# eikehmueller/IncompressibleEulerHDG

Measured on AMD Instinct MI355X. Metric: million DOF-updates/sec (HDG-IMEX k=2, 1024^2 tri mesh), higher is better.
Workload: dtype f64

## Files before the change

incompressibleeulerhdg_amd/csrc/hdg_trace_tile.hpp:

```cpp
#pragma once
#include <hip/hip_runtime.h>

namespace hdg {

template <int K>
struct TraceTile {
  static constexpr int NL = Dim<K>::NL, NT = 3 * NL;
  static constexpr int TW = 16, TH = 8, NTHREADS = 256;
  static constexpr int W2 = TW + 4, H2 = TH + 4, N2 = W2 * H2;
  static constexpr int WPE_POST = K == 1 ? 5 : (K == 2 ? 4 : (K == 3 ? 3 : 1));
  static constexpr int W3 = TW + 6, H3 = TH + 6, N3 = W3 * H3;
  static constexpr int W1 = TW + 2, H1 = TH + 2, N1 = W1 * H1;
  static constexpr int KMAX = (N2 + NTHREADS - 1) / NTHREADS;
};

template <int K, int RW, int RH>
__device__ __forceinline__ void lds_trace_stencil(const double* __restrict__ A, int li, int lj, bool in_x, bool in_y, bool below,
                                                  bool left, const DevTables& T, double* own, double* yH, double* yV, double* yD) {
  constexpr int NL = Dim<K>::NL, NT = 3 * NL;
  auto at = [&](int t, int m, int dj, int di) { return A[((t * NL + m) * RH + (lj + dj)) * RW + (li + di)]; };
  double uA[NT], uB[NT], uC[NT];
#pragma unroll
  for (int m = 0; m < NL; m++) {
    own[m] = at(0, m, 0, 0); own[NL + m] = at(2, m, 0, 0); own[2 * NL + m] = at(1, m, 0, 0);
    uA[m] = at(0, m, 1, 0); uA[2 * NL + m] = at(1, m, 0, 1);
    uB[NL + m] = at(2, m, -1, 0); uB[2 * NL + m] = at(1, m, -1, 1);
    uC[m] = at(0, m, 1, -1); uC[NL + m] = at(2, m, 0, -1);
    yH[m] = yV[m] = yD[m] = 0.0;
  }
  const bool vL = in_x && in_y, vB = in_x && below, vW = in_y && left;
#pragma unroll
  for (int m = 0; m < NL; m++) {
    if (!in_x) own[m] = 0.0;
    if (!vL) own[NL + m] = 0.0;
    if (!in_y) own[2 * NL + m] = 0.0;
    uA[NL + m] = own[NL + m];
    uB[m] = own[m];
    uC[2 * NL + m] = own[2 * NL + m];
  }
  const double* __restrict__ SL = T.SK[0];
  const double* __restrict__ SU = T.SK[1];
  if (vL) {
    mv_acc_ld<NL, NT>(SL + 0 * NL * NT, NT, own, yH, -1.0);
    mv_acc_ld<NL, NT>(SL + 1 * NL * NT, NT, own, yD, -1.0);
    mv_acc_ld<NL, NT>(SL + 2 * NL * NT, NT, own, yV, -1.0);
    mv_acc_ld<NL, NT>(SU + 1 * NL * NT, NT, uA, yD, -1.0);
  }
  if (vB) mv_acc_ld<NL, NT>(SU + 0 * NL * NT, NT, uB, yH, -1.0);
  if (vW) mv_acc_ld<NL, NT>(SU + 2 * NL * NT, NT, uC, yV, -1.0);
}

#define HDG_TILE_OF_BLOCK                                              \
  const int tiles_per_xcd_ = (int)(gridDim.x >> 3);                    \
  const int tile_v = (int)(blockIdx.x & 7) * tiles_per_xcd_ + (int)(blockIdx.x >> 3); \
  if (tile_v >= ntx * nty) return;                                     \
  const int tile_y = tile_v / ntx, tile_x = tile_v - tile_y * ntx;
struct CornerInfo {
  bool exists, in_x, in_y, below, left;
  bool own_x;
  int vH, vV;
  long o;
};
struct TileRows {
  int jlo, jhi, rlo, rhi;
};
__device__ __forceinline__ CornerInfo corner_info(const Geo& g, const TileRows& tr, int i, int j) {
  CornerInfo c;
  const int gj = g.joff + j;
  if (g.px) {
    c.exists = gj >= 0 && gj <= g.nyg && j >= tr.rlo && j < tr.rhi;
    c.own_x = i >= 0 && i < g.nx;
    const int iw = i < 0 ? i + g.nx : (i >= g.nx ? i - g.nx : i);
    c.in_x = c.exists;
    c.in_y = c.exists && gj < g.nyg;
    c.below = gj > 0;
    c.left = true;
    c.vH = gj == 0 ? 1 : (gj == g.nyg ? 2 : 0);
    c.vV = 0;
    c.o = (long)(j + GH) * g.P + iw;
    return c;
  }
  c.exists = i >= 0 && i <= g.nx && gj >= 0 && gj <= g.nyg && j >= tr.rlo && j < tr.rhi;
  c.own_x = true;
  c.in_x = c.exists && i < g.nx;
  c.in_y = c.exists && gj < g.nyg;
  c.below = gj > 0;
  c.left = i > 0;
  c.vH = gj == 0 ? 1 : (gj == g.nyg ? 2 : 0);
  c.vV = i == 0 ? 1 : (i == g.nx ? 2 : 0);
  c.o = (long)(j + GH) * g.P + i;
  return c;
}
template <int NL>
__device__ __forceinline__ void load_corner(const double* __restrict__ v, const Geo& g, const CornerInfo& c, double* e) {
#pragma unroll
  for (int m = 0; m < NL; m++) {
    e[m] = c.in_x ? v[((long)0 * NL + m) * g.G + c.o] : 0.0;
    e[NL + m] = (c.in_x && c.in_y) ? v[((long)2 * NL + m) * g.G + c.o] : 0.0;
    e[2 * NL + m] = c.in_y ? v[((long)1 * NL + m) * g.G + c.o] : 0.0;
  }
}
template <int NL>
__device__ __forceinline__ void store_corner(double* __restrict__ v, const Geo& g, const CornerInfo& c, const double* e) {
#pragma unroll
  for (int m = 0; m < NL; m++) {
    v[((long)0 * NL + m) * g.G + c.o] = c.in_x ? e[m] : 0.0;
    v[((long)2 * NL + m) * g.G + c.o] = (c.in_x && c.in_y) ? e[NL + m] : 0.0;
    v[((long)1 * NL + m) * g.G + c.o] = c.in_y ? e[2 * NL + m] : 0.0;
  }
}
template <int NL>
__device__ __forceinline__ void corner_dinv(const DevTables& T, const CornerInfo& c, double sc, const double* r, double* z) {
#pragma unroll
  for (int q = 0; q < 3 * NL; q++) z[q] = 0.0;
  mv_acc_ld<NL, NL>(T.trDinv[0][0], NL, r, z, sc);
  mv_acc_ld<NL, NL>(T.trDinv[2][0], NL, r + NL, z + NL, sc);
  mv_acc_ld<NL, NL>(T.trDinv[1][0], NL, r + 2 * NL, z + 2 * NL, sc);
  if (c.vH != 0) {
#pragma unroll
    for (int q = 0; q < NL; q++) z[q] = 0.0;
    mv_acc_ld<NL, NL>(T.trDinv[0][c.vH], NL, r, z, sc);
  }
  if (c.vV != 0) {
#pragma unroll
    for (int q = 0; q < NL; q++) z[2 * NL + q] = 0.0;
    mv_acc_ld<NL, NL>(T.trDinv[1][c.vV], NL, r + 2 * NL, z + 2 * NL, sc);
  }
}
template <int NL>
__device__ __forceinline__ int plane_of(int q) { return q < NL ? q : (q < 2 * NL ? 2 * NL + (q - NL) : NL + (q - 2 * NL)); }

template <int K>
__global__ __launch_bounds__(TraceTile<K>::NTHREADS) void k_trace_pre_tile(int ntx, int nty, Geo g, TileRows tr, DevTables T, const double* __restrict__ r, double c0, double c1,
                                                         double c2, double* __restrict__ z_out, double* __restrict__ res_out) {
  typedef TraceTile<K> TT;
  constexpr int NL = TT::NL, NT = TT::NT, TW = TT::TW, TH = TT::TH, W2 = TT::W2, H2 = TT::H2, W1 = TT::W1, H1 = TT::H1, KMAX = TT::KMAX;
  __shared__ double Ds[NT * TT::N2];
  __shared__ double Zs[NT * TT::N1];
  HDG_TILE_OF_BLOCK
  const int i0 = tile_x * TW, j0 = tr.jlo + tile_y * TH;
  double rr[KMAX][NT], dd[KMAX][NT];
#pragma unroll
  for (int k = 0; k < KMAX; k++) {
    const int idx = threadIdx.x + k * TT::NTHREADS;
    if (idx < TT::N2) {
      const int lj = idx / W2, li = idx - lj * W2;
      const int jc = j0 - 2 + lj;
      const CornerInfo c = corner_info(g, tr, i0 - 2 + li, jc);
      load_corner<NL>(r, g, c, rr[k]);
      corner_dinv<NL>(T, c, c0, rr[k], dd[k]);
#pragma unroll
      for (int q = 0; q < NT; q++) Ds[(plane_of<NL>(q) * H2 + lj) * W2 + li] = dd[k][q];
    }
  }
  __syncthreads();
#pragma unroll
  for (int k = 0; k < KMAX; k++) {
    const int idx = threadIdx.x + k * TT::NTHREADS;
    if (idx < TT::N2) {
      const int lj = idx / W2, li = idx - lj * W2;
      if (li >= 1 && li < W2 - 1 && lj >= 1 && lj < H2 - 1) {
        const int jc = j0 - 2 + lj;
        const CornerInfo c = corner_info(g, tr, i0 - 2 + li, jc);
        double z[NT];
#pragma unroll
        for (int q = 0; q < NT; q++) z[q] = 0.0;
        if (c.exists) {
          double own[NT], y[3][NL], r1[NT], zz[NT];
          lds_trace_stencil<K, W2, H2>(Ds, li, lj, c.in_x, c.in_y, c.below, c.left, T, own, y[0], y[1], y[2]);
#pragma unroll
          for (int m = 0; m < NL; m++) {
            r1[m] = rr[k][m] - y[0][m];
            r1[NL + m] = rr[k][NL + m] - y[2][m];
            r1[2 * NL + m] = rr[k][2 * NL + m] - y[1][m];
          }
          corner_dinv<NL>(T, c, c2, r1, zz);
#pragma unroll
          for (int q = 0; q < NT; q++) z[q] = dd[k][q] + fma(c1, dd[k][q], zz[q]);
        }
#pragma unroll
        for (int q = 0; q < NT; q++) Zs[(plane_of<NL>(q) * H1 + (lj - 1)) * W1 + (li - 1)] = z[q];
        if (c.exists && c.own_x && li >= 2 && li < W2 - 2 && lj >= 2 && lj < H2 - 2 && jc < tr.jhi) store_corner<NL>(z_out, g, c, z);
      }
    }
  }
  __syncthreads();
#pragma unroll
  for (int k = 0; k < KMAX; k++) {
    const int idx = threadIdx.x + k * TT::NTHREADS;
    if (idx < TT::N2) {
      const int lj = idx / W2, li = idx - lj * W2;
      if (li >= 2 && li < W2 - 2 && lj >= 2 && lj < H2 - 2) {
        const int jc = j0 - 2 + lj;
        const CornerInfo c = corner_info(g, tr, i0 - 2 + li, jc);
        if (c.exists && c.own_x && jc < tr.jhi) {
          double own[NT], y[3][NL], res[NT];
          lds_trace_stencil<K, W1, H1>(Zs, li - 1, lj - 1, c.in_x, c.in_y, c.below, c.left, T, own, y[0], y[1], y[2]);
#pragma unroll
          for (int m = 0; m < NL; m++) {
            res[m] = rr[k][m] - y[0][m];
            res[NL + m] = rr[k][NL + m] - y[2][m];
            res[2 * NL + m] = rr[k][2 * NL + m] - y[1][m];
          }
          store_corner<NL>(res_out, g, c, res);
        }
      }
    }
  }
}

template <int K, bool DOTS>
__global__ __launch_bounds__(TraceTile<K>::NTHREADS) __attribute__((amdgpu_waves_per_eu(TraceTile<K>::WPE_POST))) void k_trace_post_tile(int ntx, int nty, Geo g, TileRows tr, DevTables T, const double* __restrict__ z_in, const double* __restrict__ r,
                                                          const double* __restrict__ xc, double sH, double sV, double sD, double c0,
                                                          double c1, double c2, double* __restrict__ z_out, double* __restrict__ w_out,
                                                          double* __restrict__ part) {
  typedef TraceTile<K> TT;
  constexpr int NL = TT::NL, NT = TT::NT, TW = TT::TW, TH = TT::TH, W2 = TT::W2, H2 = TT::H2, W3 = TT::W3, H3 = TT::H3, KMAX = TT::KMAX;
  __shared__ double Zs[NT * TT::N3];
  __shared__ double Ds[NT * TT::N2];
  HDG_TILE_OF_BLOCK
  const int i0 = tile_x * TW, j0 = tr.jlo + tile_y * TH;
  const int st = g.nx + 1;
  for (int idx = threadIdx.x; idx < TT::N3; idx += TT::NTHREADS) {
    const int lj = idx / W3, li = idx - lj * W3;
    const int i = i0 - 3 + li, j = j0 - 3 + lj;
    const CornerInfo c = corner_info(g, tr, i, j);
    double z[NT];
    load_corner<NL>(z_in, g, c, z);
    if (c.exists && g.px) {
      const int n = g.nx, m = g.nx, jg = g.pj0 + j;
      const int iw = i < 0 ? i + n : (i >= n ? i - n : i), i1 = iw + 1 == n ? 0 : iw + 1;
      const int jw = jg < 0 ? jg + m : (jg >= m ? jg - m : jg), j1 = jw + 1 == m ? 0 : jw + 1;
      const double v00 = xc[(long)jw * n + iw], v10 = xc[(long)jw * n + i1], v01 = xc[(long)j1 * n + iw];
      edge_prolong(v00, v10, sH, z);
      if (c.in_y) edge_prolong(v10, v01, sD, z + NL);
      if (c.in_y) edge_prolong(v00, v01, sV, z + 2 * NL);
    } else if (c.exists) {
      const long J = g.joff + j;
      const double v00 = xc[J * st + i];
      const double v10 = c.in_x ? xc[J * st + i + 1] : 0.0, v01 = c.in_y ? xc[(J + 1) * st + i] : 0.0;
      if (c.in_x) edge_prolong(v00, v10, sH, z);
      if (c.in_x && c.in_y) edge_prolong(v10, v01, sD, z + NL);
      if (c.in_y) edge_prolong(v00, v01, sV, z + 2 * NL);
    }
#pragma unroll
    for (int q = 0; q < NT; q++) Zs[(plane_of<NL>(q) * H3 + lj) * W3 + li] = z[q];
  }
  double r0[KMAX][NT];
#pragma unroll
  for (int k = 0; k < KMAX; k++) {
    const int idx = threadIdx.x + k * TT::NTHREADS;
    const int lj = idx / W2, li = idx - lj * W2;
    CornerInfo c = corner_info(g, tr, i0 - 2 + li, j0 - 2 + lj);
    if (idx >= TT::N2) c.in_x = c.in_y = false;
    load_corner<NL>(r, g, c, r0[k]);
  }
  __syncthreads();
  double dots[5] = {0.0, 0.0, 0.0, 0.0, 0.0};
#pragma unroll
  for (int k = 0; k < KMAX; k++) {
    const int idx = threadIdx.x + k * TT::NTHREADS;
    if (idx < TT::N2) {
      const int lj = idx / W2, li = idx - lj * W2;
      const int jc = j0 - 2 + lj;
      const CornerInfo c = corner_info(g, tr, i0 - 2 + li, jc);
      double d0[NT];
#pragma unroll
      for (int q = 0; q < NT; q++) d0[q] = 0.0;
      if (c.exists) {
        double own[NT], y[3][NL];
        lds_trace_stencil<K, W3, H3>(Zs, li + 1, lj + 1, c.in_x, c.in_y, c.below, c.left, T, own, y[0], y[1], y[2]);
#pragma unroll
        for (int m = 0; m < NL; m++) {
          r0[k][m] -= y[0][m];
          r0[k][NL + m] -= y[2][m];
          r0[k][2 * NL + m] -= y[1][m];
        }
        corner_dinv<NL>(T, c, c0, r0[k], d0);
      }
#pragma unroll
      for (int q = 0; q < NT; q++) Ds[(plane_of<NL>(q) * H2 + lj) * W2 + li] = d0[q];
    }
  }
  __syncthreads();
#pragma unroll
  for (int k = 0; k < KMAX; k++) {
    const int idx = threadIdx.x + k * TT::NTHREADS;
    if (idx < TT::N2) {
      const int lj = idx / W2, li = idx - lj * W2;
      if (li >= 1 && li < W2 - 1 && lj >= 1 && lj < H2 - 1) {
        const int jc = j0 - 2 + lj;
        const CornerInfo c = corner_info(g, tr, i0 - 2 + li, jc);
        double z2[NT];
#pragma unroll
        for (int q = 0; q < NT; q++) z2[q] = 0.0;
        if (c.exists) {
          double own[NT], y[3][NL], r1[NT], zz[NT];
          lds_trace_stencil<K, W2, H2>(Ds, li, lj, c.in_x, c.in_y, c.below, c.left, T, own, y[0], y[1], y[2]);
#pragma unroll
          for (int m = 0; m < NL; m++) {
            r1[m] = r0[k][m] - y[0][m];
            r1[NL + m] = r0[k][NL + m] - y[2][m];
            r1[2 * NL + m] = r0[k][2 * NL + m] - y[1][m];
          }
          corner_dinv<NL>(T, c, c2, r1, zz);
#pragma unroll
          for (int q = 0; q < NT; q++) {
            const double z1 = Zs[(plane_of<NL>(q) * H3 + (lj + 1)) * W3 + (li + 1)] + own[q];
            z2[q] = z1 + fma(c1, own[q], zz[q]);
          }
        }
#pragma unroll
        for (int q = 0; q < NT; q++) Zs[(plane_of<NL>(q) * H3 + (lj + 1)) * W3 + (li + 1)] = z2[q];
        if (c.exists && c.own_x && li >= 2 && li < W2 - 2 && lj >= 2 && lj < H2 - 2 && jc < tr.jhi) store_corner<NL>(z_out, g, c, z2);
      }
    }
  }
  if (!w_out) return;
  double rr3[KMAX][NT];
  if (DOTS) {
#pragma unroll
    for (int k = 0; k < KMAX; k++) {
      const int idx = threadIdx.x + k * TT::NTHREADS;
      const int lj = idx / W2, li = idx - lj * W2;
      const int jc = j0 - 2 + lj;
      CornerInfo c = corner_info(g, tr, i0 - 2 + li, jc);
      if (!(idx < TT::N2 && li >= 2 && li < W2 - 2 && lj >= 2 && lj < H2 - 2 && c.exists && c.own_x && jc < tr.jhi)) c.in_x = c.in_y = false;
      load_corner<NL>(r, g, c, rr3[k]);
    }
  }
  __syncthreads();
#pragma unroll
  for (int k = 0; k < KMAX; k++) {
    const int idx = threadIdx.x + k * TT::NTHREADS;
    if (idx < TT::N2) {
      const int lj = idx / W2, li = idx - lj * W2;
      if (li >= 2 && li < W2 - 2 && lj >= 2 && lj < H2 - 2) {
        const int jc = j0 - 2 + lj;
        const CornerInfo c = corner_info(g, tr, i0 - 2 + li, jc);
        if (c.exists && c.own_x && jc < tr.jhi) {
          double own[NT], y[3][NL], w[NT];
          lds_trace_stencil<K, W3, H3>(Zs, li + 1, lj + 1, c.in_x, c.in_y, c.below, c.left, T, own, y[0], y[1], y[2]);
#pragma unroll
          for (int m = 0; m < NL; m++) { w[m] = y[0][m]; w[NL + m] = y[2][m]; w[2 * NL + m] = y[1][m]; }
          store_corner<NL>(w_out, g, c, w);
          if (DOTS) {
            const double* rr = rr3[k];
            dots[0] += sH * own[0] + sD * own[NL] + sV * own[2 * NL];
            dots[4] += sH * rr[0] + sD * rr[NL] + sV * rr[2 * NL];
#pragma unroll
            for (int q = 0; q < NT; q++) {
              const double zq = own[q];
              dots[1] = fma(zq, rr[q], dots[1]);
              dots[2] = fma(zq, zq, dots[2]);
              dots[3] = fma(zq, w[q], dots[3]);
            }
          }
        }
      }
    }
  }
  if (DOTS) {
    __shared__ double sm[TT::NTHREADS / 64][5];
    const int lane = threadIdx.x & 63, wv = threadIdx.x >> 6;
#pragma unroll
    for (int q = 0; q < 5; q++) {
      const double sv = wave_sum(dots[q]);
      if (lane == 0) sm[wv][q] = sv;
    }
    __syncthreads();
    if (threadIdx.x < 5) {
      double sv = 0.0;
      for (int w2 = 0; w2 < TT::NTHREADS / 64; w2++) sv += sm[w2][threadIdx.x];
      part[(long)threadIdx.x * (ntx * nty) + tile_v] = sv;
    }
  }
}

}
```

Before: 830.6.

## Remap tile corners to threads interior-first so inner stages use whole waves

Replaces the row-major halo-region-to-thread mapping with an interior-first, then ring-1, then ring-2 ordering, one corner per thread (N2=240 fits in 256 threads). Later stages, which only touch the halo-1 or interior region, now sit in contiguous waves, and whole waves that have no work skip a stage through a wave-uniform check. The per-thread KMAX arrays and their loops are dropped, which may lower register pressure. The dot-product reduction is rerouted through LDS in row-major order, presumably to keep the summation order deterministic, at the cost of an extra barrier and LDS traffic.

```diff
diff --git a/incompressibleeulerhdg_amd/csrc/hdg_tile_map.hpp b/incompressibleeulerhdg_amd/csrc/hdg_tile_map.hpp
--- /dev/null
+++ b/incompressibleeulerhdg_amd/csrc/hdg_tile_map.hpp
@@ -0,0 +1,34 @@
+#pragma once
+
+namespace hdg {
+
+template <int K>
+struct TileShape {
+  static constexpr int TW = 16, TH = 8;
+};
+
+struct TileCorner {
+  int li, lj;
+};
+
+template <int TW, int TH>
+constexpr TileCorner ring_corner(int r, int p) {
+  const int w = TW + 2 * r, h = TH + 2 * r, o = 2 - r;
+  if (p < 2 * w) {
+    const int top = p >= w ? 1 : 0;
+    return TileCorner{o + p - top * w, o + top * (h - 1)};
+  }
+  p -= 2 * w;
+  const int right = p >= h - 2 ? 1 : 0;
+  return TileCorner{o + right * (w - 1), o + 1 + p - right * (h - 2)};
+}
+
+template <int TW, int TH>
+constexpr TileCorner tile_corner(int idx) {
+  constexpr int N0 = TW * TH, N1 = (TW + 2) * (TH + 2);
+  if (idx < N0) return TileCorner{2 + idx % TW, 2 + idx / TW};
+  if (idx < N1) return ring_corner<TW, TH>(1, idx - N0);
+  return ring_corner<TW, TH>(2, idx - N1);
+}
+
+}
diff --git a/incompressibleeulerhdg_amd/csrc/hdg_trace_tile.hpp b/incompressibleeulerhdg_amd/csrc/hdg_trace_tile.hpp
--- a/incompressibleeulerhdg_amd/csrc/hdg_trace_tile.hpp
+++ b/incompressibleeulerhdg_amd/csrc/hdg_trace_tile.hpp
@@ -1,17 +1,33 @@
 #pragma once
 #include <hip/hip_runtime.h>
+
+#include "hdg_tile_map.hpp"
 
 namespace hdg {
 
 template <int K>
 struct TraceTile {
   static constexpr int NL = Dim<K>::NL, NT = 3 * NL;
-  static constexpr int TW = 16, TH = 8, NTHREADS = 256;
+  static constexpr int TW = TileShape<K>::TW, TH = TileShape<K>::TH, NTHREADS = 256;
+  static constexpr int N0 = TW * TH;
   static constexpr int W2 = TW + 4, H2 = TH + 4, N2 = W2 * H2;
   static constexpr int WPE_POST = K == 1 ? 5 : (K == 2 ? 4 : (K == 3 ? 3 : 1));
   static constexpr int W3 = TW + 6, H3 = TH + 6, N3 = W3 * H3;
   static constexpr int W1 = TW + 2, H1 = TH + 2, N1 = W1 * H1;
-  static constexpr int KMAX = (N2 + NTHREADS - 1) / NTHREADS;
+  static_assert(N2 <= NTHREADS && N3 <= 2 * NTHREADS, "one corner of the halo-2 region per thread, two trips over the halo-3 region");
+};
+
+template <int K>
+struct TileWave {
+  int idx, li, lj;
+  int first;
+  __device__ __forceinline__ TileWave() {
+    idx = (int)threadIdx.x;
+    first = __builtin_amdgcn_readfirstlane(idx) & ~63;
+    const TileCorner c = tile_corner<TraceTile<K>::TW, TraceTile<K>::TH>(idx);
+    li = c.li; lj = c.lj;
+  }
+  __device__ __forceinline__ bool runs(int n) const { return first < n; }
 };
 
 template <int K, int RW, int RH>
@@ -134,77 +150,57 @@
 __global__ __launch_bounds__(TraceTile<K>::NTHREADS) void k_trace_pre_tile(int ntx, int nty, Geo g, TileRows tr, DevTables T, const double* __restrict__ r, double c0, double c1,
                                                          double c2, double* __restrict__ z_out, double* __restrict__ res_out) {
   typedef TraceTile<K> TT;
-  constexpr int NL = TT::NL, NT = TT::NT, TW = TT::TW, TH = TT::TH, W2 = TT::W2, H2 = TT::H2, W1 = TT::W1, H1 = TT::H1, KMAX = TT::KMAX;
+  constexpr int NL = TT::NL, NT = TT::NT, TW = TT::TW, TH = TT::TH, W2 = TT::W2, H2 = TT::H2, W1 = TT::W1, H1 = TT::H1;
   __shared__ double Ds[NT * TT::N2];
   __shared__ double Zs[NT * TT::N1];
   HDG_TILE_OF_BLOCK
   const int i0 = tile_x * TW, j0 = tr.jlo + tile_y * TH;
-  double rr[KMAX][NT], dd[KMAX][NT];
-#pragma unroll
-  for (int k = 0; k < KMAX; k++) {
-    const int idx = threadIdx.x + k * TT::NTHREADS;
-    if (idx < TT::N2) {
-      const int lj = idx / W2, li = idx - lj * W2;
-      const int jc = j0 - 2 + lj;
-      const CornerInfo c = corner_info(g, tr, i0 - 2 + li, jc);
-      load_corner<NL>(r, g, c, rr[k]);
-      corner_dinv<NL>(T, c, c0, rr[k], dd[k]);
-#pragma unroll
-      for (int q = 0; q < NT; q++) Ds[(plane_of<NL>(q) * H2 + lj) * W2 + li] = dd[k][q];
-    }
-  }
-  __syncthreads();
-#pragma unroll
-  for (int k = 0; k < KMAX; k++) {
-    const int idx = threadIdx.x + k * TT::NTHREADS;
-    if (idx < TT::N2) {
-      const int lj = idx / W2, li = idx - lj * W2;
-      if (li >= 1 && li < W2 - 1 && lj >= 1 && lj < H2 - 1) {
-        const int jc = j0 - 2 + lj;
-        const CornerInfo c = corner_info(g, tr, i0 - 2 + li, jc);
-        double z[NT];
-#pragma unroll
-        for (int q = 0; q < NT; q++) z[q] = 0.0;
-        if (c.exists) {
-          double own[NT], y[3][NL], r1[NT], zz[NT];
-          lds_trace_stencil<K, W2, H2>(Ds, li, lj, c.in_x, c.in_y, c.below, c.left, T, own, y[0], y[1], y[2]);
-#pragma unroll
-          for (int m = 0; m < NL; m++) {
-            r1[m] = rr[k][m] - y[0][m];
-            r1[NL + m] = rr[k][NL + m] - y[2][m];
-            r1[2 * NL + m] = rr[k][2 * NL + m] - y[1][m];
-          }
-          corner_dinv<NL>(T, c, c2, r1, zz);
-#pragma unroll
-          for (int q = 0; q < NT; q++) z[q] = dd[k][q] + fma(c1, dd[k][q], zz[q]);
+  const TileWave<K> tw;
+  const int idx = tw.idx, li = tw.li, lj = tw.lj, jc = j0 - 2 + lj;
+  const CornerInfo c = corner_info(g, tr, i0 - 2 + li, jc);
+  double rr[NT], dd[NT];
+  if (idx < TT::N2) {
+    load_corner<NL>(r, g, c, rr);
+    corner_dinv<NL>(T, c, c0, rr, dd);
+#pragma unroll
+    for (int q = 0; q < NT; q++) Ds[(plane_of<NL>(q) * H2 + lj) * W2 + li] = dd[q];
+  }
+  __syncthreads();
+  if (tw.runs(TT::N1)) {
+    if (idx < TT::N1) {
+      double z[NT];
+#pragma unroll
+      for (int q = 0; q < NT; q++) z[q] = 0.0;
+      if (c.exists) {
+        double own[NT], y[3][NL], r1[NT], zz[NT];
+        lds_trace_stencil<K, W2, H2>(Ds, li, lj, c.in_x, c.in_y, c.below, c.left, T, own, y[0], y[1], y[2]);
+#pragma unroll
+        for (int m = 0; m < NL; m++) {
+          r1[m] = rr[m] - y[0][m];
+          r1[NL + m] = rr[NL + m] - y[2][m];
+          r1[2 * NL + m] = rr[2 * NL + m] - y[1][m];
         }
-#pragma unroll
-        for (int q = 0; q < NT; q++) Zs[(plane_of<NL>(q) * H1 + (lj - 1)) * W1 + (li - 1)] = z[q];
-        if (c.exists && c.own_x && li >= 2 && li < W2 - 2 && lj >= 2 && lj < H2 - 2 && jc < tr.jhi) store_corner<NL>(z_out, g, c, z);
-      }
-    }
-  }
-  __syncthreads();
-#pragma unroll
-  for (int k = 0; k < KMAX; k++) {
-    const int idx = threadIdx.x + k * TT::NTHREADS;
-    if (idx < TT::N2) {
-      const int lj = idx / W2, li = idx - lj * W2;
-      if (li >= 2 && li < W2 - 2 && lj >= 2 && lj < H2 - 2) {
-        const int jc = j0 - 2 + lj;
-        const CornerInfo c = corner_info(g, tr, i0 - 2 + li, jc);
-        if (c.exists && c.own_x && jc < tr.jhi) {
-          double own[NT], y[3][NL], res[NT];
-          lds_trace_stencil<K, W1, H1>(Zs, li - 1, lj - 1, c.in_x, c.in_y, c.below, c.left, T, own, y[0], y[1], y[2]);
-#pragma unroll
-          for (int m = 0; m < NL; m++) {
-            res[m] = rr[k][m] - y[0][m];
-            res[NL + m] = rr[k][NL + m] - y[2][m];
-            res[2 * NL + m] = rr[k][2 * NL + m] - y[1][m];
-          }
-          store_corner<NL>(res_out, g, c, res);
-        }
-      }
+        corner_dinv<NL>(T, c, c2, r1, zz);
+#pragma unroll
+        for (int q = 0; q < NT; q++) z[q] = dd[q] + fma(c1, dd[q], zz[q]);
+      }
+#pragma unroll
+      for (int q = 0; q < NT; q++) Zs[(plane_of<NL>(q) * H1 + (lj - 1)) * W1 + (li - 1)] = z[q];
+      if (c.exists && c.own_x && idx < TT::N0 && jc < tr.jhi) store_corner<NL>(z_out, g, c, z);
+    }
+  }
+  __syncthreads();
+  if (tw.runs(TT::N0)) {
+    if (idx < TT::N0 && c.exists && c.own_x && jc < tr.jhi) {
+      double own[NT], y[3][NL], res[NT];
+      lds_trace_stencil<K, W1, H1>(Zs, li - 1, lj - 1, c.in_x, c.in_y, c.below, c.left, T, own, y[0], y[1], y[2]);
+#pragma unroll
+      for (int m = 0; m < NL; m++) {
+        res[m] = rr[m] - y[0][m];
+        res[NL + m] = rr[NL + m] - y[2][m];
+        res[2 * NL + m] = rr[2 * NL + m] - y[1][m];
+      }
+      store_corner<NL>(res_out, g, c, res);
     }
   }
 }
@@ -215,14 +211,20 @@
                                                           double c1, double c2, double* __restrict__ z_out, double* __restrict__ w_out,
                                                           double* __restrict__ part) {
   typedef TraceTile<K> TT;
-  constexpr int NL = TT::NL, NT = TT::NT, TW = TT::TW, TH = TT::TH, W2 = TT::W2, H2 = TT::H2, W3 = TT::W3, H3 = TT::H3, KMAX = TT::KMAX;
+  constexpr int NL = TT::NL, NT = TT::NT, TW = TT::TW, TH = TT::TH, W2 = TT::W2, H2 = TT::H2, W3 = TT::W3, H3 = TT::H3;
   __shared__ double Zs[NT * TT::N3];
   __shared__ double Ds[NT * TT::N2];
   HDG_TILE_OF_BLOCK
   const int i0 = tile_x * TW, j0 = tr.jlo + tile_y * TH;
   const int st = g.nx + 1;
-  for (int idx = threadIdx.x; idx < TT::N3; idx += TT::NTHREADS) {
-    const int lj = idx / W3, li = idx - lj * W3;
+  const TileWave<K> tw;
+  const int idx = tw.idx;
+  constexpr int REST = TT::N3 - TT::NTHREADS;
+#pragma unroll
+  for (int trip = 0; trip < 2; trip++) {
+    const int idx3 = idx + trip * REST;
+    if (trip == 1 && idx3 < TT::NTHREADS) continue;
+    const int lj = idx3 / W3, li = idx3 - lj * W3;
     const int i = i0 - 3 + li, j = j0 - 3 + lj;
     const CornerInfo c = corner_info(g, tr, i, j);
     double z[NT];
@@ -246,135 +248,115 @@
 #pragma unroll
     for (int q = 0; q < NT; q++) Zs[(plane_of<NL>(q) * H3 + lj) * W3 + li] = z[q];
   }
-  double r0[KMAX][NT];
-#pragma unroll
-  for (int k = 0; k < KMAX; k++) {
-    const int idx = threadIdx.x + k * TT::NTHREADS;
-    const int lj = idx / W2, li = idx - lj * W2;
-    CornerInfo c = corner_info(g, tr, i0 - 2 + li, j0 - 2 + lj);
-    if (idx >= TT::N2) c.in_x = c.in_y = false;
-    load_corner<NL>(r, g, c, r0[k]);
+  const int li = tw.li, lj = tw.lj, jc = j0 - 2 + lj;
+  const CornerInfo c = corner_info(g, tr, i0 - 2 + li, jc);
+  double r0[NT];
+  {
+    CornerInfo cl = c;
+    if (idx >= TT::N2) cl.in_x = cl.in_y = false;
+    load_corner<NL>(r, g, cl, r0);
   }
   __syncthreads();
   double dots[5] = {0.0, 0.0, 0.0, 0.0, 0.0};
-#pragma unroll
-  for (int k = 0; k < KMAX; k++) {
-    const int idx = threadIdx.x + k * TT::NTHREADS;
-    if (idx < TT::N2) {
-      const int lj = idx / W2, li = idx - lj * W2;
-      const int jc = j0 - 2 + lj;
-      const CornerInfo c = corner_info(g, tr, i0 - 2 + li, jc);
-      double d0[NT];
-#pragma unroll
-      for (int q = 0; q < NT; q++) d0[q] = 0.0;
+  if (idx < TT::N2) {
+    double d0[NT];
+#pragma unroll
+    for (int q = 0; q < NT; q++) d0[q] = 0.0;
+    if (c.exists) {
+      double own[NT], y[3][NL];
+      lds_trace_stencil<K, W3, H3>(Zs, li + 1, lj + 1, c.in_x, c.in_y, c.below, c.left, T, own, y[0], y[1], y[2]);
+#pragma unroll
+      for (int m = 0; m < NL; m++) {
+        r0[m] -= y[0][m];
+        r0[NL + m] -= y[2][m];
+        r0[2 * NL + m] -= y[1][m];
+      }
+      corner_dinv<NL>(T, c, c0, r0, d0);
+    }
+#pragma unroll
+    for (int q = 0; q < NT; q++) Ds[(plane_of<NL>(q) * H2 + lj) * W2 + li] = d0[q];
+  }
+  __syncthreads();
+  if (tw.runs(TT::N1)) {
+    if (idx < TT::N1) {
+      double z2[NT];
+#pragma unroll
+      for (int q = 0; q < NT; q++) z2[q] = 0.0;
       if (c.exists) {
-        double own[NT], y[3][NL];
-        lds_trace_stencil<K, W3, H3>(Zs, li + 1, lj + 1, c.in_x, c.in_y, c.below, c.left, T, own, y[0], y[1], y[2]);
+        double own[NT], y[3][NL], r1[NT], zz[NT];
+        lds_trace_stencil<K, W2, H2>(Ds, li, lj, c.in_x, c.in_y, c.below, c.left, T, own, y[0], y[1], y[2]);
 #pragma unroll
         for (int m = 0; m < NL; m++) {
-          r0[k][m] -= y[0][m];
-          r0[k][NL + m] -= y[2][m];
-          r0[k][2 * NL + m] -= y[1][m];
+          r1[m] = r0[m] - y[0][m];
+          r1[NL + m] = r0[NL + m] - y[2][m];
+          r1[2 * NL + m] = r0[2 * NL + m] - y[1][m];
         }
-        corner_dinv<NL>(T, c, c0, r0[k], d0);
-      }
-#pragma unroll
-      for (int q = 0; q < NT; q++) Ds[(plane_of<NL>(q) * H2 + lj) * W2 + li] = d0[q];
-    }
-  }
-  __syncthreads();
-#pragma unroll
-  for (int k = 0; k < KMAX; k++) {
-    const int idx = threadIdx.x + k * TT::NTHREADS;
-    if (idx < TT::N2) {
-      const int lj = idx / W2, li = idx - lj * W2;
-      if (li >= 1 && li < W2 - 1 && lj >= 1 && lj < H2 - 1) {
-        const int jc = j0 - 2 + lj;
-        const CornerInfo c = corner_info(g, tr, i0 - 2 + li, jc);
-        double z2[NT];
-#pragma unroll
-        for (int q = 0; q < NT; q++) z2[q] = 0.0;
-        if (c.exists) {
-          double own[NT], y[3][NL], r1[NT], zz[NT];
-          lds_trace_stencil<K, W2, H2>(Ds, li, lj, c.in_x, c.in_y, c.below, c.left, T, own, y[0], y[1], y[2]);
-#pragma unroll
-          for (int m = 0; m < NL; m++) {
-            r1[m] = r0[k][m] - y[0][m];
-            r1[NL + m] = r0[k][NL + m] - y[2][m];
-            r1[2 * NL + m] = r0[k][2 * NL + m] - y[1][m];
-          }
-          corner_dinv<NL>(T, c, c2, r1, zz);
-#pragma unroll
-          for (int q = 0; q < NT; q++) {
-            const double z1 = Zs[(plane_of<NL>(q) * H3 + (lj + 1)) * W3 + (li + 1)] + own[q];
-            z2[q] = z1 + fma(c1, own[q], zz[q]);
-          }
+        corner_dinv<NL>(T, c, c2, r1, zz);
+#pragma unroll
+        for (int q = 0; q < NT; q++) {
+          const double z1 = Zs[(plane_of<NL>(q) * H3 + (lj + 1)) * W3 + (li + 1)] + own[q];
+          z2[q] = z1 + fma(c1, own[q], zz[q]);
         }
-#pragma unroll
-        for (int q = 0; q < NT; q++) Zs[(plane_of<NL>(q) * H3 + (lj + 1)) * W3 + (li + 1)] = z2[q];
-        if (c.exists && c.own_x && li >= 2 && li < W2 - 2 && lj >= 2 && lj < H2 - 2 && jc < tr.jhi) store_corner<NL>(z_out, g, c, z2);
-      }
+      }
+#pragma unroll
+      for (int q = 0; q < NT; q++) Zs[(plane_of<NL>(q) * H3 + (lj + 1)) * W3 + (li + 1)] = z2[q];
+      if (c.exists && c.own_x && idx < TT::N0 && jc < tr.jhi) store_corner<NL>(z_out, g, c, z2);
     }
   }
   if (!w_out) return;
-  double rr3[KMAX][NT];
-  if (DOTS) {
-#pragma unroll
-    for (int k = 0; k < KMAX; k++) {
-      const int idx = threadIdx.x + k * TT::NTHREADS;
-      const int lj = idx / W2, li = idx - lj * W2;
-      const int jc = j0 - 2 + lj;
-      CornerInfo c = corner_info(g, tr, i0 - 2 + li, jc);
-      if (!(idx < TT::N2 && li >= 2 && li < W2 - 2 && lj >= 2 && lj < H2 - 2 && c.exists && c.own_x && jc < tr.jhi)) c.in_x = c.in_y = false;
-      load_corner<NL>(r, g, c, rr3[k]);
-    }
-  }
-  __syncthreads();
-#pragma unroll
-  for (int k = 0; k < KMAX; k++) {
-    const int idx = threadIdx.x + k * TT::NTHREADS;
-    if (idx < TT::N2) {
-      const int lj = idx / W2, li = idx - lj * W2;
-      if (li >= 2 && li < W2 - 2 && lj >= 2 && lj < H2 - 2) {
-        const int jc = j0 - 2 + lj;
-        const CornerInfo c = corner_info(g, tr, i0 - 2 + li, jc);
-        if (c.exists && c.own_x && jc < tr.jhi) {
-          double own[NT], y[3][NL], w[NT];
-          lds_trace_stencil<K, W3, H3>(Zs, li + 1, lj + 1, c.in_x, c.in_y, c.below, c.left, T, own, y[0], y[1], y[2]);
-#pragma unroll
-          for (int m = 0; m < NL; m++) { w[m] = y[0][m]; w[NL + m] = y[2][m]; w[2 * NL + m] = y[1][m]; }
-          store_corner<NL>(w_out, g, c, w);
-          if (DOTS) {
-            const double* rr = rr3[k];
-            dots[0] += sH * own[0] + sD * own[NL] + sV * own[2 * NL];
-            dots[4] += sH * rr[0] + sD * rr[NL] + sV * rr[2 * NL];
-#pragma unroll
-            for (int q = 0; q < NT; q++) {
-              const double zq = own[q];
-              dots[1] = fma(zq, rr[q], dots[1]);
-              dots[2] = fma(zq, zq, dots[2]);
-              dots[3] = fma(zq, w[q], dots[3]);
-            }
-          }
+  const bool run3 = tw.runs(TT::N0);
+  const bool live3 = idx < TT::N0 && c.exists && c.own_x && jc < tr.jhi;
+  double rr3[NT];
+  if (DOTS && run3) {
+    CornerInfo cl = c;
+    if (!live3) cl.in_x = cl.in_y = false;
+    load_corner<NL>(r, g, cl, rr3);
+  }
+  __syncthreads();
+  if (run3) {
+    if (live3) {
+      double own[NT], y[3][NL], w[NT];
+      lds_trace_stencil<K, W3, H3>(Zs, li + 1, lj + 1, c.in_x, c.in_y, c.below, c.left, T, own, y[0], y[1], y[2]);
+#pragma unroll
+      for (int m = 0; m < NL; m++) { w[m] = y[0][m]; w[NL + m] = y[2][m]; w[2 * NL + m] = y[1][m]; }
+      store_corner<NL>(w_out, g, c, w);
+      if (DOTS) {
+        const double* rr = rr3;
+        dots[0] += sH * own[0] + sD * own[NL] + sV * own[2 * NL];
+        dots[4] += sH * rr[0] + sD * rr[NL] + sV * rr[2 * NL];
+#pragma unroll
+        for (int q = 0; q < NT; q++) {
+          const double zq = own[q];
+          dots[1] = fma(zq, rr[q], dots[1]);
+          dots[2] = fma(zq, zq, dots[2]);
+          dots[3] = fma(zq, w[q], dots[3]);
         }
       }
     }
   }
   if (DOTS) {
     __shared__ double sm[TT::NTHREADS / 64][5];
-    const int lane = threadIdx.x & 63, wv = threadIdx.x >> 6;
+    static_assert(NT >= 5, "Ds holds five values per corner");
+    const int lane = idx & 63, wv = idx >> 6;
+    if (idx < TT::N0) {
+#pragma unroll
+      for (int q = 0; q < 5; q++) Ds[q * TT::N2 + lj * W2 + li] = dots[q];
+    }
+    __syncthreads();
+    const int sj = idx / W2, si = idx - sj * W2;
+    const bool in_tile = si >= 2 && si < W2 - 2 && sj >= 2 && sj < H2 - 2;
 #pragma unroll
     for (int q = 0; q < 5; q++) {
-      const double sv = wave_sum(dots[q]);
+      const double sv = wave_sum(in_tile ? Ds[q * TT::N2 + idx] : 0.0);
       if (lane == 0) sm[wv][q] = sv;
     }
     __syncthreads();
-    if (threadIdx.x < 5) {
+    if (idx < 5) {
       double sv = 0.0;
-      for (int w2 = 0; w2 < TT::NTHREADS / 64; w2++) sv += sm[w2][threadIdx.x];
-      part[(long)threadIdx.x * (ntx * nty) + tile_v] = sv;
-    }
-  }
-}
-
-}
+      for (int w2 = 0; w2 < TT::NTHREADS / 64; w2++) sv += sm[w2][idx];
+      part[(long)idx * (ntx * nty) + tile_v] = sv;
+    }
+  }
+}
+
+}
```

New measurement: 835.8, median of 6. Within noise of the previous version (+0.6%).
